# i2Nav-WHU/IC-GVINS

Hardware: AMD Instinct MI355X
Metric: frames/s at 1280x720, 300 feats, 10-KF window; residual/Jacobian eval/s (higher is better)
Workload: dtype u8/int64 front-end (f32/f64 solves), f64 factors

## Files before the change

ic-gvins_amd/csrc/ctx.hip:

```cpp
#include <cstdarg>

#include <sys/prctl.h>
#include <time.h>

#include "icg_internal.h"

int icg_fail(icg_ctx *ctx, int code, const char *fmt, ...) {
    char buf[512];
    va_list ap;
    va_start(ap, fmt);
    vsnprintf(buf, sizeof buf, fmt, ap);
    va_end(ap);
    if (ctx) ctx->err = buf;
    return code;
}

int icg_hip_check(icg_ctx *ctx, hipError_t e, const char *what) {
    if (e == hipSuccess) return 0;
    return icg_fail(ctx, ICG_ERR_HIP, "HIP error %d (%s) at %s", (int) e, hipGetErrorString(e), what);
}

static thread_local std::string g_create_error;

extern "C" const char *icg_version(void) { return "icgvins-hip 0.1 (gfx950)"; }

extern "C" const char *icg_last_error(const icg_ctx *ctx) { return ctx ? ctx->err.c_str() : g_create_error.c_str(); }

int icg_stream_wait_poll(icg_ctx *ctx) {
    static thread_local bool slack_set = false;
    if (!slack_set) {
        (void) prctl(PR_SET_TIMERSLACK, 1000UL, 0, 0, 0);
        slack_set = true;
    }
    struct timespec ts = {0, ctx->poll_sleep_ns};
    for (int it = 0;; it++) {
        hipError_t e = hipStreamQuery(ctx->stream);
        if (e == hipSuccess) return ICG_OK;
        if (e != hipErrorNotReady) return icg_hip_check(ctx, e, "hipStreamQuery");
        if (it >= 4) nanosleep(&ts, nullptr);
    }
}

extern "C" int icg_ctx_set_wait_mode(icg_ctx *ctx, int mode, int sleep_us) {
    if (!ctx || (mode != ICG_WAIT_SPIN && mode != ICG_WAIT_POLL) || (mode == ICG_WAIT_POLL && sleep_us <= 0)) return ICG_ERR_INVALID;
    if (ctx->wait_mode_env) return ICG_OK;
    ctx->poll_sleep_ns = mode == ICG_WAIT_POLL ? 1000L * sleep_us : 0;
    return ICG_OK;
}

icg_pyr_desc icg_make_pyr_desc(const icg_ctx *ctx) {
    icg_pyr_desc d{};
    d.base       = ctx->d_frames;
    d.slot_bytes = ctx->slot_bytes;
    d.n_levels   = ctx->n_levels;
    for (int l = 0; l < ICG_MAX_LEVELS; l++) {
        d.w[l]     = ctx->lv[l].w;
        d.h[l]     = ctx->lv[l].h;
        d.pitch[l] = ctx->lv[l].pitch;
        d.off[l]   = (unsigned int) ctx->lv[l].off;
    }
    return d;
}

extern "C" int icg_ctx_create(const icg_ctx_config *cfg, icg_ctx **out) {
    if (!cfg || !out) return ICG_ERR_INVALID;
    *out = nullptr;
    if (cfg->width < 32 || cfg->height < 32 || cfg->n_slots < 1 || cfg->max_batch < 1 || cfg->max_points < 1) {
        g_create_error = "icg_ctx_create: invalid configuration";
        return ICG_ERR_INVALID;
    }
    int ndev = 0;
    if (hipGetDeviceCount(&ndev) != hipSuccess || ndev <= 0 || cfg->device >= ndev) {
        g_create_error = "icg_ctx_create: no HIP device available (this library has no CPU fallback)";
        return ICG_ERR_NODEVICE;
    }
    icg_ctx *ctx = new icg_ctx();
    ctx->cfg     = *cfg;
    int rc       = 0;
    auto bail    = [&](int code) {
        g_create_error = ctx->err;
        icg_ctx_destroy(ctx);
        return code;
    };
    if ((rc = icg_hip_check(ctx, hipSetDevice(cfg->device), "hipSetDevice"))) return bail(rc);
    if ((rc = icg_hip_check(ctx, hipStreamCreateWithFlags(&ctx->stream, hipStreamNonBlocking), "hipStreamCreate")))
        return bail(rc);

    {
        const char *wm = getenv("ICG_WAIT_MODE");
        if (wm && strncmp(wm, "poll", 4) == 0) ctx->poll_sleep_ns = (wm[4] == ':' ? atol(wm + 5) : 20) * 1000L;
        ctx->wait_mode_env = wm != nullptr;
        if (wm && strcmp(wm, "block") == 0 &&
            (rc = icg_hip_check(ctx, hipEventCreateWithFlags(&ctx->ev_wait, hipEventBlockingSync | hipEventDisableTiming), "hipEventCreate")))
            return bail(rc);
    }

    int w = cfg->width, h = cfg->height;
    size_t off    = 0;
    ctx->n_levels = 0;
    for (int l = 0; l < ICG_MAX_LEVELS; l++) {
        if (l > 0) {
            w = (w + 1) / 2;
            h = (h + 1) / 2;
            if (w <= ICG_LK_WIN || h <= ICG_LK_WIN) break;
        }
        ctx->lv[l].w     = w;
        ctx->lv[l].h     = h;
        ctx->lv[l].pitch = (int) icg_align_up((size_t) w, 128);
        ctx->lv[l].off   = off;
        off += icg_align_up((size_t) ctx->lv[l].pitch * h, 256);
        ctx->n_levels++;
    }
    ctx->slot_bytes = off;
    for (int l = 0; l + 1 < ctx->n_levels; l++)
        if (ctx->lv[l].pitch % 4 != 0 || ctx->lv[l].off % 4 != 0 || ctx->lv[l].off + (size_t) ctx->lv[l].pitch * ctx->lv[l].h + 8 > ctx->slot_bytes ||
            ctx->lv[l].w < 8 || ctx->lv[l].h < 6 || ctx->lv[l].pitch < 16) {
            ctx->err = "icg_ctx_create: pyramid layout does not meet the row-stream kernel's invariants";
            return bail(ICG_ERR_INVALID);
        }
    ctx->raw_pitch  = ctx->lv[0].pitch;
    size_t tiles2   = (size_t) ICG_CLAHE_TILES * ICG_CLAHE_TILES;
    if ((rc = icg_hip_check(ctx, hipMalloc(&ctx->d_frames, ctx->slot_bytes * (size_t) cfg->n_slots), "hipMalloc frames")))
        return bail(rc);
    if ((rc = icg_hip_check(ctx, hipMalloc(&ctx->d_raw, (size_t) ctx->raw_pitch * cfg->height * cfg->max_batch),
                            "hipMalloc raw")))
        return bail(rc);
    if ((rc = icg_hip_check(ctx, hipMalloc(&ctx->d_lut, tiles2 * 256 * cfg->max_batch), "hipMalloc lut")))
        return bail(rc);
    if ((rc = icg_hip_check(ctx, hipMalloc(&ctx->d_histmean, sizeof(double) * cfg->max_batch), "hipMalloc hist")))
        return bail(rc);
    size_t want = (size_t) cfg->max_points * 96 + (size_t) cfg->max_factors * (48 + 16) * 8 + (1u << 20);
    if ((rc = icg_arena_reserve(ctx, want))) return bail(rc);
    *out = ctx;
    return ICG_OK;
}

extern "C" void icg_ctx_destroy(icg_ctx *ctx) {
    if (!ctx) return;
    (void) hipSetDevice(ctx->cfg.device);
    if (ctx->stream) (void) hipStreamSynchronize(ctx->stream);
    for (auto e : ctx->ev_pool) (void) hipEventDestroy(e);
    if (ctx->ev_wait) (void) hipEventDestroy(ctx->ev_wait);
    void *dev[] = {ctx->d_frames, ctx->d_raw,     ctx->d_bgr,  ctx->d_lut,      ctx->d_histmean,
                   ctx->d_roi_max, ctx->d_cand, ctx->d_cand_cnt, ctx->d_arena,    ctx->d_obs,
                   ctx->d_fidx,   ctx->d_rJ,      ctx->d_params,   ctx->d_sys,
                   ctx->d_fwin,   ctx->d_lmwin,   ctx->marg.d_J,   ctx->marg.d_e0,  ctx->marg.d_x0,
                   ctx->marg.d_meta, ctx->d_lin_scratch};
    for (void *p : dev)
        if (p) (void) hipFree(p);
    for (icg_partition *pt : {&ctx->part_1, &ctx->part_w}) {
        if (pt->plan.d_buf) (void) hipFree(pt->plan.d_buf);
        if (pt->plan.d_part) (void) hipFree(pt->plan.d_part);
    }

    if (ctx->h_arena) (void) hipHostFree(ctx->h_arena);
    if (ctx->h_fstage) (void) hipHostFree(ctx->h_fstage);
    if (ctx->stream) (void) hipStreamDestroy(ctx->stream);
    delete ctx;
}

extern "C" int icg_ctx_sync(icg_ctx *ctx) {
    if (!ctx) return ICG_ERR_INVALID;
    ICG_HIP(ctx, hipStreamSynchronize(ctx->stream));
    icg_prof_collect(ctx);
    return ICG_OK;
}

extern "C" void *icg_ctx_stream(icg_ctx *ctx) { return ctx ? (void *) ctx->stream : nullptr; }

extern "C" int icg_set_camera(icg_ctx *ctx, const icg_camera *cam) {
    if (!ctx || !cam) return ICG_ERR_INVALID;
    ctx->cam     = *cam;
    ctx->has_cam = true;
    return ICG_OK;
}

extern "C" int icg_pyramid_levels(const icg_ctx *ctx) { return ctx ? ctx->n_levels : 0; }

int icg_arena_reserve(icg_ctx *ctx, size_t bytes) {
    if (bytes <= ctx->arena_cap) return 0;
    if (ctx->arena_off != 0) return icg_fail(ctx, ICG_ERR_NOMEM, "arena grow requested mid-call");
    size_t cap = icg_align_up(bytes + bytes / 2, 1 << 16);
    ICG_HIP(ctx, hipStreamSynchronize(ctx->stream));
    if (ctx->h_arena) (void) hipHostFree(ctx->h_arena);
    if (ctx->d_arena) (void) hipFree(ctx->d_arena);
    ctx->h_arena = nullptr;
    ctx->d_arena = nullptr;
    ctx->arena_cap = 0;
    ICG_HIP(ctx, hipHostMalloc((void **) &ctx->h_arena, cap, hipHostMallocDefault));
    ICG_HIP(ctx, hipMalloc((void **) &ctx->d_arena, cap));
    ctx->arena_cap = cap;
    return 0;
}

int icg_arena_drain(icg_ctx *ctx) {
    if (ctx->arena_inflight == 0) return 0;
    int rc = icg_hip_check(ctx, hipStreamSynchronize(ctx->stream), "hipStreamSynchronize");
    ctx->arena_inflight = 0;
    ctx->arena_off      = 0;
    return rc;
}

size_t icg_arena_alloc(icg_ctx *ctx, size_t bytes) {
    size_t off = icg_align_up(ctx->arena_off, 256);
    if (off + bytes > ctx->arena_cap) {
        ctx->arena_overflow = true;
        off                 = 0;
        if (bytes > ctx->arena_cap) abort();
    } else {
        ctx->arena_off = off + bytes;
    }
    return off;
}

int icg_arena_overflow_check(icg_ctx *ctx) {
    if (!ctx->arena_overflow) return 0;
    ctx->arena_overflow = false;
    ctx->arena_off      = 0;
    return icg_fail(ctx, ICG_ERR_NOMEM, "staging arena overflow: the entry point reserved too little");
}

int icg_arena_h2d(icg_ctx *ctx, size_t begin, size_t end) {
    if (end <= begin) return 0;
    ICG_HIP(ctx, hipMemcpyAsync(ctx->d_arena + begin, ctx->h_arena + begin, end - begin, hipMemcpyHostToDevice,
                                ctx->stream));
    return 0;
}
int icg_arena_d2h(icg_ctx *ctx, size_t begin, size_t end) {
    if (end <= begin) return 0;
    ICG_HIP(ctx, hipMemcpyAsync(ctx->h_arena + begin, ctx->d_arena + begin, end - begin, hipMemcpyDeviceToHost,
                                ctx->stream));
    return 0;
}

static hipEvent_t prof_event(icg_ctx *ctx) {
    if (ctx->ev_used == ctx->ev_pool.size()) {
        hipEvent_t e;
        if (hipEventCreate(&e) != hipSuccess) return nullptr;
        ctx->ev_pool.push_back(e);
// ... 79 lines not shown
```

ic-gvins_amd/csrc/icg_internal.h:

```cpp
#pragma once
#include <utility>
#include <hip/hip_runtime.h>

#include <cstdint>
#include <cstdio>
#include <cstring>
#include <map>
#include <string>
#include <vector>

#include "../../include/icgvins_hip.h"

#define ICG_MAX_LEVELS 4
#define ICG_LK_WIN 21
#define ICG_LK_HALF 10
#define ICG_CLAHE_TILES 21

struct icg_level {
    int w, h, pitch;
    size_t off;
};

struct icg_prof_rec {
    int launches  = 0;
    double total_ms = 0;
};

struct icg_asm_plan {
    int n_runs = 0, Kmax = 1;
    std::vector<int32_t> run_off;
    std::vector<int32_t> pose_off;
    std::vector<int32_t> pose_glob;
    char *d_buf = nullptr;
    size_t buf_cap = 0;
    int32_t *d_perm = nullptr;
    int32_t *d_runs = nullptr;
    int32_t *d_run_off = nullptr;
    int32_t *d_pair_run = nullptr;
    int32_t *d_lrec = nullptr;
    int32_t *d_lm_foff = nullptr;
    double *d_part = nullptr;
    size_t part_cap = 0;
};
struct icg_partition {
    int W = 0;
    bool plan_valid = false;
    std::vector<int32_t> fac_off, lm_off;
    std::vector<int64_t> sys_off;
    std::vector<double> damp;
    int sys_P = 0, sys_valid = 0;
    icg_asm_plan plan;
};

struct icg_marg_set {
    int n = 0, n_blocks = 0;
    int64_t total_r = 0, total_x = 0, total_j = 0, total_jac = 0, max_jac = 0;
    double *d_J = nullptr;
    double *d_e0 = nullptr, *d_x0 = nullptr;
    char *d_meta = nullptr;
    size_t J_cap = 0, e0_cap = 0, x0_cap = 0, meta_cap = 0;
    std::vector<int64_t> h_meta;
};

struct icg_ctx {
    icg_ctx_config cfg{};
    hipStream_t stream = nullptr;
    std::string err;
    hipEvent_t ev_wait = nullptr;
    bool wait_mode_env = false;
    long poll_sleep_ns = 0;

    int n_levels = 0;
    icg_level lv[ICG_MAX_LEVELS]{};
    size_t slot_bytes = 0;
    uint8_t *d_frames = nullptr;

    int raw_pitch      = 0;
    uint8_t *d_raw     = nullptr;
    uint8_t *d_bgr     = nullptr;
    uint8_t *d_lut     = nullptr;
    double *d_histmean = nullptr;

    uint32_t *d_roi_max   = nullptr;
    unsigned long long *d_cand = nullptr;
    int32_t *d_cand_cnt   = nullptr;
    int roi_state_cap     = 0;
    size_t cand_cap_per_roi = 0;

    char *h_arena = nullptr;
    char *d_arena = nullptr;
    size_t arena_cap = 0, arena_off = 0;
    size_t arena_inflight = 0;
    bool arena_overflow = false;

    double *d_obs = nullptr;
    int32_t *d_fidx = nullptr;
    int n_factors_resident = 0, factors_cap = 0;
    double *d_rJ = nullptr;
    int rJ_valid = 0, rJ_has_jac = 0;
    double *d_params = nullptr;
    size_t params_cap = 0;
    int last_n_poses = 0, last_n_lm = 0;
    double last_huber = 0.0;
    std::vector<int32_t> h_fidx;
    char *h_fstage = nullptr;
    size_t fstage_cap = 0;
    int fstage_n = -1;
    double *d_sys = nullptr;
    size_t sys_cap = 0;
    double sys_min_diag = 0.0, sys_max_diag = 0.0;
    icg_partition part_1, part_w;
    int32_t *d_fwin = nullptr;
    int32_t *d_lmwin = nullptr;
    int lmwin_cap = 0;

    icg_marg_set marg;
    double *d_lin_scratch = nullptr;
    size_t lin_scratch_cap = 0;

    icg_camera cam{};
    bool has_cam = false;

    bool prof_on = false;
    std::vector<hipEvent_t> ev_pool;
    size_t ev_used = 0;
    struct pending {
        std::string name;
        hipEvent_t a, b;
    };
    std::vector<pending> prof_pending;
    std::map<std::string, icg_prof_rec> prof;
};

int icg_fail(icg_ctx *ctx, int code, const char *fmt, ...);
int icg_hip_check(icg_ctx *ctx, hipError_t e, const char *what);
#define ICG_HIP(ctx, call)                                                                                             \
    do {                                                                                                               \
        int _rc = icg_hip_check((ctx), (call), #call);                                                                 \
        if (_rc) return _rc;                                                                                           \
    } while (0)

int icg_arena_reserve(icg_ctx *ctx, size_t bytes);
static inline size_t icg_align_up(size_t v, size_t a) { return (v + a - 1) / a * a; }
size_t icg_arena_alloc(icg_ctx *ctx, size_t bytes);
template <typename T> static inline T *icg_h(icg_ctx *ctx, size_t off) { return reinterpret_cast<T *>(ctx->h_arena + off); }
template <typename T> static inline T *icg_d(icg_ctx *ctx, size_t off) { return reinterpret_cast<T *>(ctx->d_arena + off); }
int icg_arena_overflow_check(icg_ctx *ctx);
int icg_arena_h2d(icg_ctx *ctx, size_t begin, size_t end);
int icg_arena_d2h(icg_ctx *ctx, size_t begin, size_t end);
int icg_arena_drain(icg_ctx *ctx);

struct icg_prof_scope {
    icg_ctx *ctx;
    hipEvent_t a = nullptr, b = nullptr;
    const char *name;
    icg_prof_scope(icg_ctx *c, const char *n);
    ~icg_prof_scope();
};
void icg_prof_collect(icg_ctx *ctx);

struct icg_pyr_desc {
    uint8_t *base;
    unsigned long long slot_bytes;
    int n_levels;
// ... 158 lines not shown
```

ic-gvins_amd/csrc/image.hip:

```cpp
#include <algorithm>

#include "icg_internal.h"

#define PRE_MAX_JOBS 64
struct pre_jobs {
    const uint8_t *src[PRE_MAX_JOBS];
    int32_t slot[PRE_MAX_JOBS];
    int stride;
    const int32_t *slot_ind;
};
__device__ __forceinline__ int pre_job_slot(const pre_jobs &j, int b) { return j.slot_ind ? j.slot_ind[b] : j.slot[b]; }

__global__ void k_bgr2gray(const uint8_t *bgr, int w, int h, int sstride, size_t sbatch, uint8_t *gray, int gstride,
                           size_t gbatch) {
    int x = blockIdx.x * blockDim.x + threadIdx.x;
    int y = blockIdx.y;
    int b = blockIdx.z;
    if (x >= w) return;
    const uint8_t *p = bgr + (size_t) b * sbatch + (size_t) y * sstride + 3 * x;
    gray[(size_t) b * gbatch + (size_t) y * gstride + x] =
        (uint8_t) ((p[0] * 1868 + p[1] * 9617 + p[2] * 4899 + 8192) >> 14);
}

__global__ void k_hist256(pre_jobs jobs, int w, int h, unsigned int *hist ) {
    __shared__ unsigned int sh[256];
    int b = blockIdx.y;
    sh[threadIdx.x] = 0;
    __syncthreads();
    const uint8_t *src = jobs.src[b];
    const int stride   = jobs.stride;
    int total          = src ? w * h : 0;
    for (int i = blockIdx.x * blockDim.x + threadIdx.x; i < total; i += gridDim.x * blockDim.x) {
        int y = i / w, x = i - y * w;
        atomicAdd(&sh[src[(size_t) y * stride + x]], 1u);
    }
    __syncthreads();
    if (sh[threadIdx.x]) atomicAdd(&hist[(size_t) b * 256 + threadIdx.x], sh[threadIdx.x]);
}

struct clahe_geom {
    int w, h, tw, th, clip;
    float lut_scale, inv_tw, inv_th;
};

__device__ __forceinline__ int wave_sum_i32(int v) {
    v += __builtin_amdgcn_update_dpp(0, v, 0xB1, 0xF, 0xF, false);
    v += __builtin_amdgcn_update_dpp(0, v, 0x4E, 0xF, 0xF, false);
    v += __builtin_amdgcn_update_dpp(0, v, 0x141, 0xF, 0xF, false);
    v += __builtin_amdgcn_update_dpp(0, v, 0x140, 0xF, 0xF, false);
    v += __builtin_amdgcn_update_dpp(0, v, 0x142, 0xA, 0xF, false);
    v += __builtin_amdgcn_update_dpp(0, v, 0x143, 0xC, 0xF, false);
    return __builtin_amdgcn_readlane(v, 63);
}
__device__ __forceinline__ int wave_scan_i32(int v) {
    v += __builtin_amdgcn_update_dpp(0, v, 0x111, 0xF, 0xF, true);
    v += __builtin_amdgcn_update_dpp(0, v, 0x112, 0xF, 0xF, true);
    v += __builtin_amdgcn_update_dpp(0, v, 0x114, 0xF, 0xF, true);
    v += __builtin_amdgcn_update_dpp(0, v, 0x118, 0xF, 0xF, true);
    v += __builtin_amdgcn_update_dpp(0, v, 0x142, 0xA, 0xF, false);
    v += __builtin_amdgcn_update_dpp(0, v, 0x143, 0xC, 0xF, false);
    return v;
}

__global__ __launch_bounds__(64) void k_clahe_lut(pre_jobs jobs, clahe_geom g, uint8_t *lut , int n_items) {
    __shared__ __attribute__((aligned(16))) unsigned int hist[256];
    const int lane = threadIdx.x;
    const int item = icg_xcd_chunked(blockIdx.x, n_items);
    if (item >= n_items) return;
    const int b    = item / (ICG_CLAHE_TILES * ICG_CLAHE_TILES);
    const int tile = item - b * (ICG_CLAHE_TILES * ICG_CLAHE_TILES);
    const int ty = tile / ICG_CLAHE_TILES, tx = tile - ty * ICG_CLAHE_TILES;
    const uint8_t *src = jobs.src[b];
    if (!src) return;
    const int stride   = jobs.stride;
    reinterpret_cast<uint4 *>(hist)[lane] = make_uint4(0, 0, 0, 0);
    __syncthreads();

    const int x_begin = tx * g.tw, x_end = x_begin + g.tw, y_begin = ty * g.th;
    const int xa  = x_begin & ~3;
    const int ndw = (((x_end + 3) & ~3) - xa) >> 2;
    const bool pad_small = g.th * ICG_CLAHE_TILES < 2 * g.h - 1;
    auto load_row_dword = [&](int r, int x) -> unsigned int {
        const uint8_t *row = src + (size_t) (pad_small ? icg_reflect1(y_begin + r, g.h) : icg_reflect101(y_begin + r, g.h)) * stride;
        if (x + 3 < g.w) return *reinterpret_cast<const unsigned int *>(row + x);
        unsigned int v = 0;
#pragma unroll
        for (int j = 0; j < 4; j++) v |= (unsigned int) row[icg_reflect101(x + j, g.w)] << (8 * j);
        return v;
    };
    const int nin = ndw - 2;
    const bool fast = nin >= 1 && nin <= 16 && y_begin + g.th <= g.h && xa + 4 * ndw <= g.w;
    if (fast) {
        const int d = lane & 15, q = lane >> 4;
        const bool on = d < nin;
        const uint8_t *p = src + (size_t) (y_begin + q) * stride + (xa + 4 * (on ? d + 1 : 1));
        unsigned char *hb = reinterpret_cast<unsigned char *>(hist);
        const size_t step = 4 * (size_t) stride;
        for (int r = q; r < g.th; r += 16, p += 4 * step) {
            unsigned int v[4];
            bool ok[4];
#pragma unroll
            for (int k = 0; k < 4; k++) {
                ok[k] = on && r + 4 * k < g.th;
                v[k]  = r + 4 * k < g.th ? *reinterpret_cast<const unsigned int *>(p + k * step) : 0u;
            }
#pragma unroll
            for (int k = 0; k < 4; k++) {
                if (ok[k]) {
                    atomicAdd(reinterpret_cast<unsigned int *>(hb + ((v[k] << 2) & 0x3fcu)), 1u);
                    atomicAdd(reinterpret_cast<unsigned int *>(hb + ((v[k] >> 6) & 0x3fcu)), 1u);
                    atomicAdd(reinterpret_cast<unsigned int *>(hb + ((v[k] >> 14) & 0x3fcu)), 1u);
                    atomicAdd(reinterpret_cast<unsigned int *>(hb + ((v[k] >> 22) & 0x3fcu)), 1u);
                }
            }
        }
    } else {
        {
            const int items = g.th * (nin > 0 ? nin : 0);
            const unsigned int magic = nin > 0 ? ((1u << 20) + (unsigned int) nin - 1u) / (unsigned int) nin : 0u;
            constexpr int CH = 9;
            for (int base = 0; base < items; base += 64 * CH) {
                unsigned int v[CH];
                bool ok[CH];
    #pragma unroll
                for (int k = 0; k < CH; k++) {
                    const int i = base + k * 64 + lane;
                    ok[k]       = i < items;
                    v[k]        = 0;
                    if (ok[k]) {
                        const int r = (int) (((unsigned int) i * magic) >> 20), d = 1 + i - r * nin;
                        v[k]        = load_row_dword(r, xa + 4 * d);
                    }
                }
    #pragma unroll
                for (int k = 0; k < CH; k++) {
                    if (ok[k]) {
    #pragma unroll
                        for (int j = 0; j < 4; j++) atomicAdd(&hist[(v[k] >> (8 * j)) & 0xff], 1u);
                    }
                }
            }
        }
    }
    {
        const int nedge = ndw >= 2 ? 2 : 1, items = g.th * nedge;
        for (int i = lane; i < items; i += 64) {
            const int r = nedge == 2 ? (i >> 1) : i, d = (nedge == 2 && (i & 1)) ? ndw - 1 : 0;
            const int x = xa + 4 * d;
            const unsigned int v = load_row_dword(r, x);
#pragma unroll
            for (int j = 0; j < 4; j++) {
                const int xx = x + j;
                if (xx >= x_begin && xx < x_end) atomicAdd(&hist[(v >> (8 * j)) & 0xff], 1u);
            }
        }
// ... 21 lines not shown
        const int t = 4 * lane + j;
        hv[j] += batch_add;
        if (residual != 0 && (t % step) == 0 && (t / step) < residual) hv[j]++;
        run += hv[j];
        hv[j] = run;
    }
    const int incl = wave_scan_i32(run);
    const int excl = incl - run;
    unsigned int packed = 0;
#pragma unroll
    for (int j = 0; j < 4; j++) {
        const float f = rintf((float) (excl + hv[j]) * g.lut_scale);
        int iv        = (int) f;
        iv            = iv < 0 ? 0 : (iv > 255 ? 255 : iv);
        packed |= (unsigned int) iv << (8 * j);
    }
    reinterpret_cast<unsigned int *>(lut + ((size_t) b * ICG_CLAHE_TILES * ICG_CLAHE_TILES + tile) * 256)[lane] = packed;
}

#define CLAHE_CHUNK 256
#define CLAHE_MAXCOLS 24
#define CLAHE_FCOLS 8

typedef float f32x2 __attribute__((ext_vector_type(2)));

template <bool FLT>
__device__ __forceinline__ void clahe_apply_body(const pre_jobs &jobs, const clahe_geom &g, const uint8_t *lut, uint8_t *frames, size_t slot_bytes,
                                                 int dpitch, unsigned int *slut, int strip, int chunk, int b, int t, int dslot, int p_lo, int npairs,
                                                 int x_begin) {
    const int T = ICG_CLAHE_TILES;
    int ty1 = strip - 1, ty2 = strip;
    if (ty1 < 0) ty1 = 0;
    if (ty2 > T - 1) ty2 = T - 1;
    const unsigned int *blut = reinterpret_cast<const unsigned int *>(lut + (size_t) b * T * T * 256);
    for (int i = t; i < npairs * 64; i += 256) {
        const int p = p_lo + (i >> 6), v4 = i & 63;
        int c1 = p - 1, c2 = p;
        if (c1 < 0) c1 = 0;
        if (c2 > T - 1) c2 = T - 1;
        const unsigned int A = blut[(ty1 * T + c1) * 64 + v4], B = blut[(ty1 * T + c2) * 64 + v4];
        const unsigned int C = blut[(ty2 * T + c1) * 64 + v4], D = blut[(ty2 * T + c2) * 64 + v4];
        if (FLT) {
            float4 *dst = reinterpret_cast<float4 *>(slut) + 4 * i;
#define CL_F(w, k) ((float) (((w) >> (8 * (k))) & 0xffu))
            dst[0] = make_float4(CL_F(A, 0), CL_F(B, 0), CL_F(C, 0), CL_F(D, 0));
            dst[1] = make_float4(CL_F(A, 1), CL_F(B, 1), CL_F(C, 1), CL_F(D, 1));
            dst[2] = make_float4(CL_F(A, 2), CL_F(B, 2), CL_F(C, 2), CL_F(D, 2));
            dst[3] = make_float4(CL_F(A, 3), CL_F(B, 3), CL_F(C, 3), CL_F(D, 3));
#undef CL_F
        } else {
            const unsigned int ab01 = __builtin_amdgcn_perm(B, A, 0x05010400u), ab23 = __builtin_amdgcn_perm(B, A, 0x07030602u);
            const unsigned int cd01 = __builtin_amdgcn_perm(D, C, 0x05010400u), cd23 = __builtin_amdgcn_perm(D, C, 0x07030602u);
            uint4 e;
            e.x = __builtin_amdgcn_perm(cd01, ab01, 0x05040100u);
            e.y = __builtin_amdgcn_perm(cd01, ab01, 0x07060302u);
            e.z = __builtin_amdgcn_perm(cd23, ab23, 0x05040100u);
            e.w = __builtin_amdgcn_perm(cd23, ab23, 0x07060302u);
            reinterpret_cast<uint4 *>(slut)[i] = e;
        }
    }
    __syncthreads();

    const int wave = t >> 6, lane = t & 63;
    const int x0 = x_begin + lane * 4;
    int pofs[4];
    float xa[4], xa1[4];
#pragma unroll
    for (int k = 0; k < 4; k++) {
        const int x     = x0 + k;
        const float txf = x * g.inv_tw - 0.5f;
        const int tx1   = (int) floorf(txf);
        xa[k]           = txf - tx1;
        xa1[k]          = 1.0f - xa[k];
        int p           = tx1 + 1 - p_lo;
        p               = p < 0 ? 0 : (p > npairs - 1 ? npairs - 1 : p);
        pofs[k]         = p << 8;
    }
    if (x0 >= g.w) return;

    int y_lo = (strip - 1) * g.th + g.th / 2 - 2;
    int y_hi = strip * g.th + g.th / 2 + 3;
    if (y_lo < 0) y_lo = 0;
    if (y_hi > g.h) y_hi = g.h;
    const uint8_t *src = jobs.src[b];
    const int stride   = jobs.stride;
    uint8_t *dst       = frames + (size_t) dslot * slot_bytes;
    if (FLT) {
        const float4 *sf = reinterpret_cast<const float4 *>(slut);
        for (int y = y_lo + wave; y < y_hi; y += 4) {
            const float tyf = y * g.inv_th - 0.5f;
            const int tyr   = (int) floorf(tyf);
            if (tyr != strip - 1) continue;
            const float ya = tyf - tyr, ya1 = 1.0f - ya;
            const unsigned int pin = *reinterpret_cast<const unsigned int *>(src + (size_t) y * stride + x0);
            const float4 e0 = sf[pofs[0] + (pin & 0xff)], e1 = sf[pofs[1] + ((pin >> 8) & 0xff)];
            const float4 e2 = sf[pofs[2] + ((pin >> 16) & 0xff)], e3 = sf[pofs[3] + (pin >> 24)];
            const float r0 = (e0.x * xa1[0] + e0.y * xa[0]) * ya1 + (e0.z * xa1[0] + e0.w * xa[0]) * ya;
            const float r1 = (e1.x * xa1[1] + e1.y * xa[1]) * ya1 + (e1.z * xa1[1] + e1.w * xa[1]) * ya;
            const float r2 = (e2.x * xa1[2] + e2.y * xa[2]) * ya1 + (e2.z * xa1[2] + e2.w * xa[2]) * ya;
            const float r3 = (e3.x * xa1[3] + e3.y * xa[3]) * ya1 + (e3.z * xa1[3] + e3.w * xa[3]) * ya;
            const unsigned int m0 = __float_as_uint(r0 + 12582912.f), m1 = __float_as_uint(r1 + 12582912.f);
            const unsigned int m2 = __float_as_uint(r2 + 12582912.f), m3 = __float_as_uint(r3 + 12582912.f);
            const unsigned int lo = __builtin_amdgcn_perm(m1, m0, 0x0c0c0400u), hi = __builtin_amdgcn_perm(m3, m2, 0x0c0c0400u);
            *reinterpret_cast<unsigned int *>(dst + (size_t) y * dpitch + x0) = __builtin_amdgcn_perm(hi, lo, 0x05040100u);
        }
        return;
    }
    const f32x2 XA01 = {xa[0], xa[1]}, XA23 = {xa[2], xa[3]}, XB01 = {xa1[0], xa1[1]}, XB23 = {xa1[2], xa1[3]};
    for (int y = y_lo + wave; y < y_hi; y += 4) {
        const float tyf = y * g.inv_th - 0.5f;
        const int tyr   = (int) floorf(tyf);
        if (tyr != strip - 1) continue;
        const float ya = tyf - tyr, ya1 = 1.0f - ya;
        const unsigned int pin = *reinterpret_cast<const unsigned int *>(src + (size_t) y * stride + x0);
        const unsigned int e0 = slut[pofs[0] + (pin & 0xff)], e1 = slut[pofs[1] + ((pin >> 8) & 0xff)];
        const unsigned int e2 = slut[pofs[2] + ((pin >> 16) & 0xff)], e3 = slut[pofs[3] + (pin >> 24)];
#define CL_B(e, k) ((float) (((e) >> (8 * (k))) & 0xffu))
        const f32x2 A01 = {CL_B(e0, 0), CL_B(e1, 0)}, B01 = {CL_B(e0, 1), CL_B(e1, 1)};
        const f32x2 C01 = {CL_B(e0, 2), CL_B(e1, 2)}, D01 = {CL_B(e0, 3), CL_B(e1, 3)};
        const f32x2 A23 = {CL_B(e2, 0), CL_B(e3, 0)}, B23 = {CL_B(e2, 1), CL_B(e3, 1)};
        const f32x2 C23 = {CL_B(e2, 2), CL_B(e3, 2)}, D23 = {CL_B(e2, 3), CL_B(e3, 3)};
#undef CL_B
        const f32x2 r01 = (A01 * XB01 + B01 * XA01) * ya1 + (C01 * XB01 + D01 * XA01) * ya;
        const f32x2 r23 = (A23 * XB23 + B23 * XA23) * ya1 + (C23 * XB23 + D23 * XA23) * ya;
        const float res[4] = {r01.x, r01.y, r23.x, r23.y};
        unsigned int pout = 0;
#pragma unroll
        for (int k = 0; k < 4; k++) {
            const int iv = (int) rintf(res[k]);
            pout |= (unsigned int) (iv < 0 ? 0 : (iv > 255 ? 255 : iv)) << (8 * k);
        }
        *reinterpret_cast<unsigned int *>(dst + (size_t) y * dpitch + x0) = pout;
    }
}

__global__ __launch_bounds__(256) void k_clahe_apply(pre_jobs jobs, clahe_geom g, const uint8_t *lut, uint8_t *frames,
                                                     size_t slot_bytes, int dpitch) {
    __shared__ __attribute__((aligned(16))) unsigned int slut[CLAHE_FCOLS * 256 * 4];
    static_assert(CLAHE_FCOLS * 4 >= CLAHE_MAXCOLS, "the byte form must fit the same array");
    const int strip = blockIdx.x;
    const int chunk = blockIdx.y;
    const int b     = blockIdx.z;
    const int t     = threadIdx.x;
    const int dslot = pre_job_slot(jobs, b);
    if (!jobs.src[b] || dslot < 0) return;
    const int x_begin = chunk * CLAHE_CHUNK;
    int x_end         = x_begin + CLAHE_CHUNK;
    if (x_end > g.w) x_end = g.w;
    const int p_lo   = (int) floorf(x_begin * g.inv_tw - 0.5f) + 1;
    const int p_hi   = (int) floorf((x_end - 1) * g.inv_tw - 0.5f) + 1;
    const int npairs = p_hi - p_lo + 1;
    if (npairs <= CLAHE_FCOLS)
        clahe_apply_body<true>(jobs, g, lut, frames, slot_bytes, dpitch, slut, strip, chunk, b, t, dslot, p_lo, npairs, x_begin);
    else
        clahe_apply_body<false>(jobs, g, lut, frames, slot_bytes, dpitch, slut, strip, chunk, b, t, dslot, p_lo, npairs, x_begin);
}

#define PR_STRIP_OUT 128
struct pr_sel {
    unsigned int a, b, t, v;
};
typedef unsigned int pr_u3 __attribute__((ext_vector_type(3)));
__device__ __forceinline__ pr_u3 pr_load(const uint8_t *row, unsigned int wx) {
    typedef pr_u3 __attribute__((aligned(4))) u3a;
    return *reinterpret_cast<const u3a *>(row + wx);
}
template <bool EDGE> __device__ __forceinline__ unsigned int pr_hsum(const pr_u3 E, const pr_sel &S) {
    unsigned int A, B, V4;
    if (EDGE) {
        A  = __builtin_amdgcn_perm(E.y, E.x, S.a);
        B  = __builtin_amdgcn_perm(E.y, E.x, S.b);
        V4 = __builtin_amdgcn_perm(E.z, __builtin_amdgcn_perm(E.y, E.x, S.t), S.v);
    } else {
        A  = __builtin_amdgcn_alignbyte(E.y, E.x, 2);
        B  = E.y;
        V4 = E.z & 0xffu;
    }
    const unsigned int h0 = __builtin_amdgcn_udot4(B, 0x00010000u, __builtin_amdgcn_udot4(A, 0x04060401u, 0u, false), false);
    const unsigned int h1 = __builtin_amdgcn_udot4(B, 0x04060401u, V4, false);
    return h0 | (h1 << 16);
}

template <bool EDGE>
__device__ __forceinline__ void pr_band(const uint8_t *src, int sh, int spitch, uint8_t *dst, int dpitch, int i0, int i1, unsigned int wx,
                                        const pr_sel &S, unsigned int dcol, bool store) {
    auto srow = [&](int r) { return src + (unsigned int) __builtin_amdgcn_readfirstlane(icg_reflect1(r, sh) * spitch); };
    unsigned int hA = pr_hsum<EDGE>(pr_load(srow(2 * i0 - 2), wx), S), hB = pr_hsum<EDGE>(pr_load(srow(2 * i0 - 1), wx), S);
    unsigned int hC = pr_hsum<EDGE>(pr_load(srow(2 * i0), wx), S);
    pr_u3 R1 = pr_load(srow(2 * i0 + 1), wx), R2 = pr_load(srow(2 * i0 + 2), wx);
    for (int i = i0; i < i1; i++) {
        const pr_u3 N1 = pr_load(srow(2 * i + 3), wx), N2 = pr_load(srow(2 * i + 4), wx);
        const unsigned int hD = pr_hsum<EDGE>(R1, S), hE = pr_hsum<EDGE>(R2, S);
        unsigned int v = hA + hE;
        v              = ((hB + hD) << 2) + v;
        v += (hC << 2) + (hC + hC);
        v += 0x00800080u;
        if (store) *reinterpret_cast<unsigned short *>(dst + (size_t) i * dpitch + dcol) = (unsigned short) __builtin_amdgcn_perm(v, v, 0x0c0c0301u);
        hA = hC, hB = hD, hC = hE;
        R1 = N1, R2 = N2;
    }
}

__global__ __launch_bounds__(64) void k_pyrdown_rows(uint8_t *frames, size_t slot_bytes, pre_jobs jobs, unsigned int src_off, int sw, int sh,
                                                     int spitch, unsigned int dst_off, int dw, int dh, int dpitch, int n_strips, int n_bands,
                                                     int band_rows, int n_tasks) {
    const int task = icg_xcd_chunked(blockIdx.x, n_tasks);
    if (task >= n_tasks) return;
    const int per_job = n_strips * n_bands;
    const int job = task / per_job, rem = task - job * per_job;
    const int band = rem / n_strips, strip = rem - band * n_strips;
    const int dslot = __builtin_amdgcn_readfirstlane(pre_job_slot(jobs, job));
    if (dslot < 0) return;
    uint8_t *slot = frames + (size_t) dslot * slot_bytes;
    const int lane = threadIdx.x;
    const int oj   = strip * PR_STRIP_OUT + 2 * lane;
    const int x  = min(2 * oj, (sw - 1) & ~3);
    const int wx = max(x - 4, 0);
    const bool edge = strip == 0 || 2 * (strip + 1) * PR_STRIP_OUT + 4 > sw;
    pr_sel S;
    S.a = S.b = S.t = S.v = 0;
    if (edge) {
        int ix[7];
#pragma unroll
        for (int k = 0; k < 7; k++) ix[k] = min(max(icg_reflect101(x - 2 + k, sw) - wx, 0), 11);
        S.a = (unsigned int) (ix[0] & 7) | ((unsigned int) (ix[1] & 7) << 8) | ((unsigned int) (ix[2] & 7) << 16) | ((unsigned int) (ix[3] & 7) << 24);
        S.b = (unsigned int) (ix[2] & 7) | ((unsigned int) (ix[3] & 7) << 8) | ((unsigned int) (ix[4] & 7) << 16) | ((unsigned int) (ix[5] & 7) << 24);
        S.t = 0x0c0c0c00u | (unsigned int) (ix[6] & 7);
        S.v = ix[6] >= 8 ? (0x0c0c0c04u + (unsigned int) (ix[6] - 8)) : 0x0c0c0c00u;
    }
    const int i0 = band * band_rows, i1 = min(i0 + band_rows, dh);
    if (i0 >= i1) return;
    const uint8_t *src = slot + src_off;
    uint8_t *dst       = slot + dst_off;
    const bool store   = oj < dw;
    if (edge)
        pr_band<true>(src, sh, spitch, dst, dpitch, i0, i1, (unsigned int) wx, S, (unsigned int) oj, store);
    else
        pr_band<false>(src, sh, spitch, dst, dpitch, i0, i1, (unsigned int) wx, S, (unsigned int) oj, store);
}

__global__ void k_hist_mean(int n, const unsigned int *hist, int w, int h, double *mean) {
    const int k = blockIdx.x * blockDim.x + threadIdx.x;
    if (k >= n) return;
    double acc = 0;
    for (int i = 0; i < 256; i++) {
        const float hf = (float) hist[(size_t) k * 256 + i];
        acc += hf * (float) i / 256.0;
    }
    mean[k] = acc / ((double) w * h);
}

static int preprocess_impl(icg_ctx *ctx, int n, const int32_t *slots, const int32_t *d_slot_ind, const uint8_t *const *images, int stride, int channels,
                           int src_on_device, double *hist_mean, double *d_hist_mean) {
    if (!ctx || n < 0 || (n > 0 && ((!slots && !d_slot_ind) || !images))) return ICG_ERR_INVALID;
    if (n == 0) return ICG_OK;
    if (n > ctx->cfg.max_batch) return icg_fail(ctx, ICG_ERR_CAPACITY, "preprocess batch %d > max_batch %d", n, ctx->cfg.max_batch);
    if (channels != 1 && channels != 3) return icg_fail(ctx, ICG_ERR_INVALID, "channels must be 1 or 3");
    const int w = ctx->cfg.width, h = ctx->cfg.height;
    if (stride < w * channels) return icg_fail(ctx, ICG_ERR_INVALID, "stride too small");
    for (int k = 0; k < n && slots; k++)
        if (slots[k] < 0 || slots[k] >= ctx->cfg.n_slots || !images[k]) return icg_fail(ctx, ICG_ERR_INVALID, "bad slot/image %d", k);
    ICG_HIP(ctx, hipSetDevice(ctx->cfg.device));
    const bool want_hist = hist_mean || d_hist_mean;

    const int T = ICG_CLAHE_TILES;
    int ew = w, eh = h;
    if (w % T != 0 || h % T != 0) {
        ew = w + (T - w % T);
        eh = h + (T - h % T);
    }
    clahe_geom g;
    g.w = w;
    g.h = h;
    g.tw = ew / T;
    g.th = eh / T;
    int area    = g.tw * g.th;
    g.lut_scale = 255.0f / area;
    g.clip      = (int) (3.0 * area / 256);
    if (g.clip < 1) g.clip = 1;
    g.inv_tw = 1.0f / g.tw;
    g.inv_th = 1.0f / g.th;
    static_assert(ICG_CLAHE_TILES + 1 <= CLAHE_MAXCOLS, "k_clahe_apply's staged LUT must hold every interpolation column pair");

    const size_t raw_batch = (size_t) ctx->raw_pitch * h;
    hipMemcpyKind kind     = src_on_device ? hipMemcpyDeviceToDevice : hipMemcpyHostToDevice;
    unsigned int *d_hist   = nullptr;
    if (want_hist) {
        if (int rcd = icg_arena_drain(ctx)) return rcd;
        ctx->arena_off = 0;
        int rc         = icg_arena_reserve(ctx, sizeof(unsigned int) * 256 * (size_t) n + 4096);
        if (rc) return rc;
        d_hist = icg_d<unsigned int>(ctx, icg_arena_alloc(ctx, sizeof(unsigned int) * 256 * (size_t) n));
        if ((rc = icg_arena_overflow_check(ctx))) return rc;
        ICG_HIP(ctx, hipMemsetAsync(d_hist, 0, sizeof(unsigned int) * 256 * (size_t) n, ctx->stream));
    }

    for (int base = 0; base < n; base += PRE_MAX_JOBS) {
        const int m = std::min(PRE_MAX_JOBS, n - base);
        pre_jobs jobs;
        memset(&jobs, 0, sizeof jobs);
        for (int k = 0; k < m && slots; k++) jobs.slot[k] = slots[base + k];
        jobs.slot_ind = d_slot_ind ? d_slot_ind + base : nullptr;
        if (channels == 3) {
            if (!ctx->d_bgr) ICG_HIP(ctx, hipMalloc((void **) &ctx->d_bgr, (size_t) w * 3 * h * ctx->cfg.max_batch));
            for (int k = 0; k < m; k++)
                if (images[base + k])
                    ICG_HIP(ctx, hipMemcpy2DAsync(ctx->d_bgr + (size_t) (base + k) * w * 3 * h, (size_t) w * 3, images[base + k], stride,
                                                  (size_t) w * 3, h, kind, ctx->stream));
            icg_prof_scope ps(ctx, "bgr2gray");
            hipLaunchKernelGGL(k_bgr2gray, dim3((w + 255) / 256, h, m), dim3(256), 0, ctx->stream,
                               ctx->d_bgr + (size_t) base * w * 3 * h, w, h, w * 3, (size_t) w * 3 * h,
                               ctx->d_raw + (size_t) base * raw_batch, ctx->raw_pitch, raw_batch);
            for (int k = 0; k < m; k++) jobs.src[k] = images[base + k] ? ctx->d_raw + (size_t) (base + k) * raw_batch : nullptr;
            jobs.stride = ctx->raw_pitch;
        } else {
            bool direct = src_on_device && (stride % 4 == 0);
            for (int k = 0; k < m && direct; k++) direct = (((uintptr_t) images[base + k]) % 4) == 0;
            if (direct) {
                for (int k = 0; k < m; k++) jobs.src[k] = images[base + k];
                jobs.stride = stride;
            } else {
                const bool linear = stride == w && ctx->raw_pitch == w;
                for (int k = 0; k < m; k++) {
                    uint8_t *dst = ctx->d_raw + (size_t) (base + k) * raw_batch;
                    if (!images[base + k]) {
                        jobs.src[k] = nullptr;
                        continue;
                    }
                    if (linear)
                        ICG_HIP(ctx, hipMemcpyAsync(dst, images[base + k], (size_t) w * h, kind, ctx->stream));
                    else
                        ICG_HIP(ctx, hipMemcpy2DAsync(dst, ctx->raw_pitch, images[base + k], stride, w, h, kind, ctx->stream));
                    jobs.src[k] = dst;
                }
                jobs.stride = ctx->raw_pitch;
            }
        }
        if (want_hist) {
            icg_prof_scope ps(ctx, "hist256");
            hipLaunchKernelGGL(k_hist256, dim3(64, m), dim3(256), 0, ctx->stream, jobs, w, h, d_hist + (size_t) base * 256);
        }
        uint8_t *lut = ctx->d_lut + (size_t) base * T * T * 256;
        {
            icg_prof_scope ps(ctx, "clahe_lut");
            hipLaunchKernelGGL(k_clahe_lut, dim3(icg_xcd_grid(T * T * m)), dim3(64), 0, ctx->stream, jobs, g, lut, T * T * m);
        }
        {
            icg_prof_scope ps(ctx, "clahe_apply");
            hipLaunchKernelGGL(k_clahe_apply, dim3(T + 1, (w + CLAHE_CHUNK - 1) / CLAHE_CHUNK, m), dim3(256), 0, ctx->stream, jobs,
                               g, lut, ctx->d_frames, ctx->slot_bytes, ctx->lv[0].pitch);
        }
        for (int l = 1; l < ctx->n_levels; l++) {
            icg_prof_scope ps(ctx, "pyrdown_rows");
            const icg_level &a = ctx->lv[l - 1], &bb = ctx->lv[l];
            const int n_strips = (bb.w + PR_STRIP_OUT - 1) / PR_STRIP_OUT;
            const int band_rows = bb.h >= 256 ? 32 : bb.h >= 128 ? 16 : 8;
            const int n_bands   = (bb.h + band_rows - 1) / band_rows;
            const int n_tasks   = n_strips * n_bands * m;
            hipLaunchKernelGGL(k_pyrdown_rows, dim3(icg_xcd_grid(n_tasks)), dim3(64), 0, ctx->stream, ctx->d_frames, ctx->slot_bytes, jobs,
                               (unsigned int) a.off, a.w, a.h, a.pitch, (unsigned int) bb.off, bb.w, bb.h, bb.pitch, n_strips, n_bands, band_rows,
                               n_tasks);
        }
    }
    if (d_hist_mean) hipLaunchKernelGGL(k_hist_mean, dim3((n + 63) / 64), dim3(64), 0, ctx->stream, n, d_hist, w, h, d_hist_mean);
    ICG_HIP(ctx, hipGetLastError());
    if (d_hist_mean) ctx->arena_off = 0;
    if (!hist_mean) return ICG_OK;

    std::vector<unsigned int> hc((size_t) n * 256);
    ICG_HIP(ctx, hipMemcpyAsync(hc.data(), d_hist, sizeof(unsigned int) * 256 * (size_t) n, hipMemcpyDeviceToHost, ctx->stream));
    ICG_HIP(ctx, hipStreamSynchronize(ctx->stream));
    icg_prof_collect(ctx);
    for (int k = 0; k < n; k++) {
        double acc = 0;
        for (int i = 0; i < 256; i++) {
            float hf = (float) hc[(size_t) k * 256 + i];
            acc += hf * (float) i / 256.0;
        }
        hist_mean[k] = acc / ((double) w * h);
    }
    ctx->arena_off = 0;
    return ICG_OK;
}

extern "C" int icg_frames_preprocess(icg_ctx *ctx, int n, const int32_t *slots, const uint8_t *const *images, int stride, int channels,
                                     int src_on_device, double *hist_mean) {
    if (n > 0 && !slots) return ICG_ERR_INVALID;
    return preprocess_impl(ctx, n, slots, nullptr, images, stride, channels, src_on_device, hist_mean, nullptr);
}

int icg_preprocess_launch_ind(icg_ctx *ctx, int n, const int32_t *d_slot_ind, const uint8_t *const *images, int stride, int channels,
                              int src_on_device, double *d_hist_mean) {
    return preprocess_impl(ctx, n, nullptr, d_slot_ind, images, stride, channels, src_on_device, nullptr, d_hist_mean);
}

extern "C" int icg_frame_download(icg_ctx *ctx, int slot, int level, uint8_t *dst, int dst_stride) {
    if (!ctx || !dst || slot < 0 || slot >= ctx->cfg.n_slots || level < 0 || level >= ctx->n_levels) return ICG_ERR_INVALID;
    ICG_HIP(ctx, hipSetDevice(ctx->cfg.device));
    const icg_level &L = ctx->lv[level];
    if (dst_stride < L.w) return ICG_ERR_INVALID;
    ICG_HIP(ctx, hipStreamSynchronize(ctx->stream));
    ICG_HIP(ctx, hipMemcpy2D(dst, dst_stride, ctx->d_frames + (size_t) slot * ctx->slot_bytes + L.off, L.pitch, L.w, L.h,
                             hipMemcpyDeviceToHost));
    return ICG_OK;
}
```

Before: 159,300.

## Move preprocessing job tables to device memory and launch whole batch at once

Replaces the fixed 64-entry by-value kernel argument struct with device-resident src/slot arrays. Each call fills a double-buffered pinned host table, guarded by events, and copies it to the device asynchronously. The whole batch then runs in a single set of kernel launches instead of chunks of 64, with source pointers read as wave-uniform through readfirstlane. This shrinks kernel argument size and launch count for large batches, but adds an H2D copy and a possible event wait per call.

Result: slower. 157,400 (-1.2%).

```diff
diff --git a/ic-gvins_amd/csrc/ctx.hip b/ic-gvins_amd/csrc/ctx.hip
--- a/ic-gvins_amd/csrc/ctx.hip
+++ b/ic-gvins_amd/csrc/ctx.hip
@@ -65,7 +65,7 @@
 extern "C" int icg_ctx_create(const icg_ctx_config *cfg, icg_ctx **out) {
     if (!cfg || !out) return ICG_ERR_INVALID;
     *out = nullptr;
-    if (cfg->width < 32 || cfg->height < 32 || cfg->n_slots < 1 || cfg->max_batch < 1 || cfg->max_points < 1) {
+    if (cfg->width < 32 || cfg->height < 32 || cfg->n_slots < 1 || cfg->max_batch < 1 || cfg->max_batch > 65535 || cfg->max_points < 1) {
         g_create_error = "icg_ctx_create: invalid configuration";
         return ICG_ERR_INVALID;
     }
@@ -129,6 +129,15 @@
         return bail(rc);
     if ((rc = icg_hip_check(ctx, hipMalloc(&ctx->d_histmean, sizeof(double) * cfg->max_batch), "hipMalloc hist")))
         return bail(rc);
+    {
+        const size_t jobs_bytes = (sizeof(uint8_t *) + sizeof(int32_t)) * (size_t) cfg->max_batch;
+        if ((rc = icg_hip_check(ctx, hipMalloc((void **) &ctx->d_pre_jobs, jobs_bytes), "hipMalloc preprocessing jobs"))) return bail(rc);
+        for (int k = 0; k < 2; k++) {
+            if ((rc = icg_hip_check(ctx, hipHostMalloc((void **) &ctx->h_pre_jobs[k], jobs_bytes, hipHostMallocDefault), "hipHostMalloc preprocessing jobs")))
+                return bail(rc);
+            if ((rc = icg_hip_check(ctx, hipEventCreateWithFlags(&ctx->ev_pre_jobs[k], hipEventDisableTiming), "hipEventCreate"))) return bail(rc);
+        }
+    }
     size_t want = (size_t) cfg->max_points * 96 + (size_t) cfg->max_factors * (48 + 16) * 8 + (1u << 20);
     if ((rc = icg_arena_reserve(ctx, want))) return bail(rc);
     *out = ctx;
@@ -145,7 +154,7 @@
                    ctx->d_roi_max, ctx->d_cand, ctx->d_cand_cnt, ctx->d_arena,    ctx->d_obs,
                    ctx->d_fidx,   ctx->d_rJ,      ctx->d_params,   ctx->d_sys,
                    ctx->d_fwin,   ctx->d_lmwin,   ctx->marg.d_J,   ctx->marg.d_e0,  ctx->marg.d_x0,
-                   ctx->marg.d_meta, ctx->d_lin_scratch};
+                   ctx->marg.d_meta, ctx->d_lin_scratch, ctx->d_pre_jobs};
     for (void *p : dev)
         if (p) (void) hipFree(p);
     for (icg_partition *pt : {&ctx->part_1, &ctx->part_w}) {
@@ -155,6 +164,10 @@
 
     if (ctx->h_arena) (void) hipHostFree(ctx->h_arena);
     if (ctx->h_fstage) (void) hipHostFree(ctx->h_fstage);
+    for (int k = 0; k < 2; k++) {
+        if (ctx->h_pre_jobs[k]) (void) hipHostFree(ctx->h_pre_jobs[k]);
+        if (ctx->ev_pre_jobs[k]) (void) hipEventDestroy(ctx->ev_pre_jobs[k]);
+    }
     if (ctx->stream) (void) hipStreamDestroy(ctx->stream);
     delete ctx;
 }
diff --git a/ic-gvins_amd/csrc/icg_internal.h b/ic-gvins_amd/csrc/icg_internal.h
--- a/ic-gvins_amd/csrc/icg_internal.h
+++ b/ic-gvins_amd/csrc/icg_internal.h
@@ -80,6 +80,10 @@
     uint8_t *d_bgr     = nullptr;
     uint8_t *d_lut     = nullptr;
     double *d_histmean = nullptr;
+    char *d_pre_jobs        = nullptr;
+    char *h_pre_jobs[2]     = {nullptr, nullptr};
+    hipEvent_t ev_pre_jobs[2] = {nullptr, nullptr};
+    int pre_jobs_turn       = 0;
 
     uint32_t *d_roi_max   = nullptr;
     unsigned long long *d_cand = nullptr;
diff --git a/ic-gvins_amd/csrc/image.hip b/ic-gvins_amd/csrc/image.hip
--- a/ic-gvins_amd/csrc/image.hip
+++ b/ic-gvins_amd/csrc/image.hip
@@ -2,14 +2,19 @@
 
 #include "icg_internal.h"
 
-#define PRE_MAX_JOBS 64
 struct pre_jobs {
-    const uint8_t *src[PRE_MAX_JOBS];
-    int32_t slot[PRE_MAX_JOBS];
+    const uint8_t *const *src;
+    const int32_t *slot;
     int stride;
     const int32_t *slot_ind;
 };
 __device__ __forceinline__ int pre_job_slot(const pre_jobs &j, int b) { return j.slot_ind ? j.slot_ind[b] : j.slot[b]; }
+__device__ __forceinline__ const uint8_t *pre_job_src(const pre_jobs &j, int b) {
+    const unsigned long long p = (unsigned long long) (uintptr_t) j.src[b];
+    const unsigned int lo = (unsigned int) __builtin_amdgcn_readfirstlane((int) (unsigned int) p);
+    const unsigned int hi = (unsigned int) __builtin_amdgcn_readfirstlane((int) (unsigned int) (p >> 32));
+    return (const uint8_t *) (uintptr_t) (((unsigned long long) hi << 32) | lo);
+}
 
 __global__ void k_bgr2gray(const uint8_t *bgr, int w, int h, int sstride, size_t sbatch, uint8_t *gray, int gstride,
                            size_t gbatch) {
@@ -27,7 +32,7 @@
     int b = blockIdx.y;
     sh[threadIdx.x] = 0;
     __syncthreads();
-    const uint8_t *src = jobs.src[b];
+    const uint8_t *src = pre_job_src(jobs, b);
     const int stride   = jobs.stride;
     int total          = src ? w * h : 0;
     for (int i = blockIdx.x * blockDim.x + threadIdx.x; i < total; i += gridDim.x * blockDim.x) {
@@ -70,7 +75,7 @@
     const int b    = item / (ICG_CLAHE_TILES * ICG_CLAHE_TILES);
     const int tile = item - b * (ICG_CLAHE_TILES * ICG_CLAHE_TILES);
     const int ty = tile / ICG_CLAHE_TILES, tx = tile - ty * ICG_CLAHE_TILES;
-    const uint8_t *src = jobs.src[b];
+    const uint8_t *src = pre_job_src(jobs, b);
     if (!src) return;
     const int stride   = jobs.stride;
     reinterpret_cast<uint4 *>(hist)[lane] = make_uint4(0, 0, 0, 0);
@@ -258,7 +263,7 @@
     int y_hi = strip * g.th + g.th / 2 + 3;
     if (y_lo < 0) y_lo = 0;
     if (y_hi > g.h) y_hi = g.h;
-    const uint8_t *src = jobs.src[b];
+    const uint8_t *src = pre_job_src(jobs, b);
     const int stride   = jobs.stride;
     uint8_t *dst       = frames + (size_t) dslot * slot_bytes;
     if (FLT) {
@@ -319,7 +324,7 @@
     const int b     = blockIdx.z;
     const int t     = threadIdx.x;
     const int dslot = pre_job_slot(jobs, b);
-    if (!jobs.src[b] || dslot < 0) return;
+    if (!pre_job_src(jobs, b) || dslot < 0) return;
     const int x_begin = chunk * CLAHE_CHUNK;
     int x_end         = x_begin + CLAHE_CHUNK;
     if (x_end > g.w) x_end = g.w;
@@ -471,72 +476,77 @@
         ICG_HIP(ctx, hipMemsetAsync(d_hist, 0, sizeof(unsigned int) * 256 * (size_t) n, ctx->stream));
     }
 
-    for (int base = 0; base < n; base += PRE_MAX_JOBS) {
-        const int m = std::min(PRE_MAX_JOBS, n - base);
-        pre_jobs jobs;
-        memset(&jobs, 0, sizeof jobs);
-        for (int k = 0; k < m && slots; k++) jobs.slot[k] = slots[base + k];
-        jobs.slot_ind = d_slot_ind ? d_slot_ind + base : nullptr;
-        if (channels == 3) {
-            if (!ctx->d_bgr) ICG_HIP(ctx, hipMalloc((void **) &ctx->d_bgr, (size_t) w * 3 * h * ctx->cfg.max_batch));
-            for (int k = 0; k < m; k++)
-                if (images[base + k])
-                    ICG_HIP(ctx, hipMemcpy2DAsync(ctx->d_bgr + (size_t) (base + k) * w * 3 * h, (size_t) w * 3, images[base + k], stride,
-                                                  (size_t) w * 3, h, kind, ctx->stream));
-            icg_prof_scope ps(ctx, "bgr2gray");
-            hipLaunchKernelGGL(k_bgr2gray, dim3((w + 255) / 256, h, m), dim3(256), 0, ctx->stream,
-                               ctx->d_bgr + (size_t) base * w * 3 * h, w, h, w * 3, (size_t) w * 3 * h,
-                               ctx->d_raw + (size_t) base * raw_batch, ctx->raw_pitch, raw_batch);
-            for (int k = 0; k < m; k++) jobs.src[k] = images[base + k] ? ctx->d_raw + (size_t) (base + k) * raw_batch : nullptr;
+    const int turn = ctx->pre_jobs_turn;
+    ctx->pre_jobs_turn ^= 1;
+    ICG_HIP(ctx, hipEventSynchronize(ctx->ev_pre_jobs[turn]));
+    const size_t slot_at  = sizeof(uint8_t *) * (size_t) ctx->cfg.max_batch;
+    const uint8_t **h_src = reinterpret_cast<const uint8_t **>(ctx->h_pre_jobs[turn]);
+    int32_t *h_slot       = reinterpret_cast<int32_t *>(ctx->h_pre_jobs[turn] + slot_at);
+    pre_jobs jobs;
+    jobs.src      = reinterpret_cast<const uint8_t *const *>(ctx->d_pre_jobs);
+    jobs.slot     = reinterpret_cast<const int32_t *>(ctx->d_pre_jobs + slot_at);
+    jobs.slot_ind = d_slot_ind;
+    jobs.stride   = 0;
+    for (int k = 0; k < n; k++) h_slot[k] = slots ? slots[k] : 0;
+    if (channels == 3) {
+        if (!ctx->d_bgr) ICG_HIP(ctx, hipMalloc((void **) &ctx->d_bgr, (size_t) w * 3 * h * ctx->cfg.max_batch));
+        for (int k = 0; k < n; k++)
+            if (images[k])
+                ICG_HIP(ctx, hipMemcpy2DAsync(ctx->d_bgr + (size_t) k * w * 3 * h, (size_t) w * 3, images[k], stride, (size_t) w * 3, h, kind, ctx->stream));
+        icg_prof_scope ps(ctx, "bgr2gray");
+        hipLaunchKernelGGL(k_bgr2gray, dim3((w + 255) / 256, h, n), dim3(256), 0, ctx->stream, ctx->d_bgr, w, h, w * 3, (size_t) w * 3 * h, ctx->d_raw,
+                           ctx->raw_pitch, raw_batch);
+        for (int k = 0; k < n; k++) h_src[k] = images[k] ? ctx->d_raw + (size_t) k * raw_batch : nullptr;
+        jobs.stride = ctx->raw_pitch;
+    } else {
+        bool direct = src_on_device && (stride % 4 == 0);
+        for (int k = 0; k < n && direct; k++) direct = (((uintptr_t) images[k]) % 4) == 0;
+        if (direct) {
+            for (int k = 0; k < n; k++) h_src[k] = images[k];
+            jobs.stride = stride;
+        } else {
+            const bool linear = stride == w && ctx->raw_pitch == w;
+            for (int k = 0; k < n; k++) {
+                uint8_t *dst = ctx->d_raw + (size_t) k * raw_batch;
+                if (!images[k]) {
+                    h_src[k] = nullptr;
+                    continue;
+                }
+                if (linear)
+                    ICG_HIP(ctx, hipMemcpyAsync(dst, images[k], (size_t) w * h, kind, ctx->stream));
+                else
+                    ICG_HIP(ctx, hipMemcpy2DAsync(dst, ctx->raw_pitch, images[k], stride, w, h, kind, ctx->stream));
+                h_src[k] = dst;
+            }
             jobs.stride = ctx->raw_pitch;
-        } else {
-            bool direct = src_on_device && (stride % 4 == 0);
-            for (int k = 0; k < m && direct; k++) direct = (((uintptr_t) images[base + k]) % 4) == 0;
-            if (direct) {
-                for (int k = 0; k < m; k++) jobs.src[k] = images[base + k];
-                jobs.stride = stride;
-            } else {
-                const bool linear = stride == w && ctx->raw_pitch == w;
-                for (int k = 0; k < m; k++) {
-                    uint8_t *dst = ctx->d_raw + (size_t) (base + k) * raw_batch;
-                    if (!images[base + k]) {
-                        jobs.src[k] = nullptr;
-                        continue;
-                    }
-                    if (linear)
-                        ICG_HIP(ctx, hipMemcpyAsync(dst, images[base + k], (size_t) w * h, kind, ctx->stream));
-                    else
-                        ICG_HIP(ctx, hipMemcpy2DAsync(dst, ctx->raw_pitch, images[base + k], stride, w, h, kind, ctx->stream));
-                    jobs.src[k] = dst;
-                }
-                jobs.stride = ctx->raw_pitch;
-            }
-        }
-        if (want_hist) {
-            icg_prof_scope ps(ctx, "hist256");
-            hipLaunchKernelGGL(k_hist256, dim3(64, m), dim3(256), 0, ctx->stream, jobs, w, h, d_hist + (size_t) base * 256);
-        }
-        uint8_t *lut = ctx->d_lut + (size_t) base * T * T * 256;
-        {
-            icg_prof_scope ps(ctx, "clahe_lut");
-            hipLaunchKernelGGL(k_clahe_lut, dim3(icg_xcd_grid(T * T * m)), dim3(64), 0, ctx->stream, jobs, g, lut, T * T * m);
-        }
-        {
-            icg_prof_scope ps(ctx, "clahe_apply");
-            hipLaunchKernelGGL(k_clahe_apply, dim3(T + 1, (w + CLAHE_CHUNK - 1) / CLAHE_CHUNK, m), dim3(256), 0, ctx->stream, jobs,
-                               g, lut, ctx->d_frames, ctx->slot_bytes, ctx->lv[0].pitch);
-        }
-        for (int l = 1; l < ctx->n_levels; l++) {
-            icg_prof_scope ps(ctx, "pyrdown_rows");
-            const icg_level &a = ctx->lv[l - 1], &bb = ctx->lv[l];
-            const int n_strips = (bb.w + PR_STRIP_OUT - 1) / PR_STRIP_OUT;
-            const int band_rows = bb.h >= 256 ? 32 : bb.h >= 128 ? 16 : 8;
-            const int n_bands   = (bb.h + band_rows - 1) / band_rows;
-            const int n_tasks   = n_strips * n_bands * m;
-            hipLaunchKernelGGL(k_pyrdown_rows, dim3(icg_xcd_grid(n_tasks)), dim3(64), 0, ctx->stream, ctx->d_frames, ctx->slot_bytes, jobs,
-                               (unsigned int) a.off, a.w, a.h, a.pitch, (unsigned int) bb.off, bb.w, bb.h, bb.pitch, n_strips, n_bands, band_rows,
-                               n_tasks);
-        }
+        }
+    }
+    ICG_HIP(ctx, hipMemcpyAsync(ctx->d_pre_jobs, ctx->h_pre_jobs[turn], slot_at + sizeof(int32_t) * (size_t) n, hipMemcpyHostToDevice, ctx->stream));
+    ICG_HIP(ctx, hipEventRecord(ctx->ev_pre_jobs[turn], ctx->stream));
+    if (want_hist) {
+        icg_prof_scope ps(ctx, "hist256");
+        hipLaunchKernelGGL(k_hist256, dim3(64, n), dim3(256), 0, ctx->stream, jobs, w, h, d_hist);
+    }
+    uint8_t *lut = ctx->d_lut;
+    {
+        icg_prof_scope ps(ctx, "clahe_lut");
+        hipLaunchKernelGGL(k_clahe_lut, dim3(icg_xcd_grid(T * T * n)), dim3(64), 0, ctx->stream, jobs, g, lut, T * T * n);
+    }
+    {
+        icg_prof_scope ps(ctx, "clahe_apply");
+        hipLaunchKernelGGL(k_clahe_apply, dim3(T + 1, (w + CLAHE_CHUNK - 1) / CLAHE_CHUNK, n), dim3(256), 0, ctx->stream, jobs, g, lut, ctx->d_frames,
+                           ctx->slot_bytes, ctx->lv[0].pitch);
+    }
+    for (int l = 1; l < ctx->n_levels; l++) {
+        icg_prof_scope ps(ctx, "pyrdown_rows");
+        const icg_level &a = ctx->lv[l - 1], &bb = ctx->lv[l];
+        const int n_strips = (bb.w + PR_STRIP_OUT - 1) / PR_STRIP_OUT;
+        const int band_rows = bb.h >= 256 ? 32 : bb.h >= 128 ? 16 : 8;
+        const int n_bands   = (bb.h + band_rows - 1) / band_rows;
+        const int n_tasks   = n_strips * n_bands * n;
+        hipLaunchKernelGGL(k_pyrdown_rows, dim3(icg_xcd_grid(n_tasks)), dim3(64), 0, ctx->stream, ctx->d_frames, ctx->slot_bytes, jobs,
+                           (unsigned int) a.off, a.w, a.h, a.pitch, (unsigned int) bb.off, bb.w, bb.h, bb.pitch, n_strips, n_bands, band_rows,
+                           n_tasks);
     }
     if (d_hist_mean) hipLaunchKernelGGL(k_hist_mean, dim3((n + 63) / 64), dim3(64), 0, ctx->stream, n, d_hist, w, h, d_hist_mean);
     ICG_HIP(ctx, hipGetLastError());
```
